# Shadowfear36/SegHiero

Measured on AMD Instinct MI355X. Metric: images/sec at 512x512 (ResNet-50 2-level), full train step, higher is better.
Workload: dtype f32 (convolutions: exact 3-way bf16 split of every fp32 operand, 6 bf16 MFMA products, f32 accumulate; rest plain f32)

## Files before the change

seghiero_amd/csrc/conv_bf16x6.hip:

```cpp
#include "conv_x6.h"

template <int MODE, int TM, int TN, int WGM, int WGN, int OCC = 0, int SK = 0, int PROF = 0, int ACT = 0>
__global__ __launch_bounds__(64 * WGM * WGN, OCC ? OCC : ((WGM * WGN) / 4 < 2 ? 2 : (WGM * WGN) / 4)) void conv_x6_kernel(const ConvQ p) {
    constexpr int NT = 64 * WGM * WGN;
    constexpr int BM = 32 * TM * WGM, BN = 32 * TN * WGN, BK = 32;
    constexpr int A_PLANE = BM * ROWB, B_PLANE = BN * ROWB;
    constexpr int RPP = NT / 8;
    constexpr int NA = (BM + RPP - 1) / RPP, NB = (BN + RPP - 1) / RPP;
    static_assert(BM >= RPP && BN >= RPP, "tile too small for the thread count");
    extern __shared__ __attribute__((aligned(16))) unsigned char smem[];

    const int t = threadIdx.x, lane = t & 63, wave = t >> 6;
    const int wm = wave / WGN, wn = wave % WGN, l31 = lane & 31, h = lane >> 5;
    unsigned long long tk0 = 0;
    if constexpr (PROF) tk0 = __builtin_amdgcn_s_memtime();
    const unsigned nblk = (unsigned)p.tiles_m * (unsigned)p.tiles_n;
    const unsigned bid = xcd_remap(blockIdx.x, nblk);
    const int tile_n = bid % p.tiles_n, tile_m = bid / p.tiles_n;
    const int m0 = tile_m * BM, n0 = tile_n * BN;
    int cy = 0, cx = 0, Hc = p.H, Wc = p.W, oy0 = 0, ox0 = 0, nth = p.KH, ntw = p.KW, Mc = p.M, Kt = p.K;
    if constexpr (MODE == DGRAD) {
        if (p.parity) {
            cy = blockIdx.y >> 1; cx = blockIdx.y & 1;
            oy0 = (cy + p.pad) & 1; ox0 = (cx + p.pad) & 1;
// ... 685 lines not shown
    const int tx = threadIdx.x & 31, ty = threadIdx.x >> 5;
    const float* w = T.w[lo];
    float* wt = T.wt[lo];
#pragma unroll
    for (int r = ty; r < 32; r += 8) {
        const int co = co0 + r, ci = ci0 + tx;
        tile[r][tx] = (co < Cout && ci < Cin) ? w[((long long)co * taps + tap) * Cin + ci] : 0.f;
    }
    __syncthreads();
#pragma unroll
    for (int r = ty; r < 32; r += 8) {
        const int ci = ci0 + r, co = co0 + tx;
        if (ci < Cin && co < CoutP) wt[((long long)tap * Cin + ci) * CoutP + co] = tile[tx][r];
    }
}
extern "C" int sh_weight_transpose_multi(int n, const float* const* w, float* const* wt, const int* cout, const int* taps, const int* cin,
                                         void* stream) {
    if (n <= 0 || n > SH_WT_MAX || !w || !wt || !cout || !taps || !cin) return SH_EINVAL;
    WtTab T;
    T.n = n;
    long long acc = 0;
    for (int i = 0; i < n; ++i) {
        if (!w[i] || !wt[i] || cout[i] <= 0 || taps[i] <= 0 || cin[i] <= 0) return SH_EINVAL;
        T.w[i] = w[i]; T.wt[i] = wt[i]; T.cout[i] = cout[i]; T.taps[i] = taps[i]; T.cin[i] = cin[i];
        T.start[i] = acc;
        acc += (long long)taps[i] * sh_cdiv((cout[i] + 3) & ~3, 32) * sh_cdiv(cin[i], 32);
    }
    T.start[n] = acc;
    if (acc >= (1ll << 31)) return SH_EINVAL;
    weight_transpose_multi_kernel<<<(unsigned)acc, 256, 0, (hipStream_t)stream>>>(T);
    return sh_launch_status();
}

struct BnbQ { const float* y; long long ldy; const float* mean; const float* invstd; const float* scale; const float* shift; int relu; const float* out; long long ldo;
              int act; int out_bf, add_bf; };
__global__ __launch_bounds__(256) void splitk_reduce_kernel(const float* __restrict__ slab, long long ldslab, int S, long long M, int Nn,
                                                            const float* __restrict__ bias, const float* __restrict__ addend, long long ldadd,
                                                            float* __restrict__ out, long long ldc, float* __restrict__ partials, const BnbQ bnb) {
    __shared__ float red[16][64];
    __shared__ float colmean[64];
    const int t = threadIdx.x, cq = t & 15, rl = t >> 4;
    const int n = blockIdx.y * 64 + cq * 4;
    const long long row0 = (long long)blockIdx.x * 64;
    const int npr = (int)(M - row0 < 64 ? M - row0 : 64);
    f32x4 v[4];
    const bool nok = n < Nn;
    f32x4 gq = {0.f, 0.f, 0.f, 0.f};
    f32x4 b_mu = gq, b_is = gq, b_sc = gq, b_sh = gq;
    if (bnb.y != nullptr && nok) { b_mu = ld4(bnb.mean + n); b_is = ld4(bnb.invstd + n); b_sc = ld4(bnb.scale + n); b_sh = ld4(bnb.shift + n); }
#pragma unroll
    for (int k = 0; k < 4; ++k) {
        const long long m = row0 + rl + 16 * k;
        v[k] = f32x4{0.f, 0.f, 0.f, 0.f};
        if (nok && m < M) {
            for (int s2 = 0; s2 < S; ++s2) v[k] += ld4(slab + ((long long)s2 * M + m) * ldslab + n);
            f32x4 o = v[k];
            if (bias) o += ld4(bias + n);
            if (addend) o += lda4(addend, m * ldadd + n, bnb.add_bf);
            if (bnb.y != nullptr) {
                const f32x4 yv = lda4(bnb.y, m * bnb.ldy + n, bnb.act & 4);
                if (bnb.relu) {
                    const f32x4 a = bnb.out == nullptr ? yv * b_sc + b_sh
                                    : ((bnb.act & 64) ? quad_mask_load(bnb.out, m * bnb.ldo + (n >> 2)) : lda4(bnb.out, m * bnb.ldo + n, bnb.act & 8));
#pragma unroll
                    for (int j = 0; j < 4; ++j) if (!(a[j] > 0.f)) o[j] = 0.f;
                }
                v[k] = o;
                gq += o * ((yv - b_mu) * b_is);
            }
            sta4(out, m * ldc + n, o, bnb.out_bf);
        }
    }
    if (partials == nullptr) return;
    f32x4 ssum = (v[0] + v[1]) + (v[2] + v[3]);
#pragma unroll
    for (int j = 0; j < 4; ++j) red[rl][cq * 4 + j] = ssum[j];
    __syncthreads();
    if (t < 64) {
        float a = 0.f;
#pragma unroll
        for (int k = 0; k < 16; ++k) a += red[k][t];
        colmean[t] = a / (float)npr;
        if (blockIdx.y * 64 + t < Nn) partials[((long long)blockIdx.x * 2 + 0) * Nn + blockIdx.y * 64 + t] = a;
    }
    __syncthreads();
    f32x4 q = {0.f, 0.f, 0.f, 0.f};
    if (bnb.y != nullptr) q = gq;
    else {
#pragma unroll
        for (int k = 0; k < 4; ++k)
            if (row0 + rl + 16 * k < M) {
#pragma unroll
                for (int j = 0; j < 4; ++j) { const float d = v[k][j] - colmean[cq * 4 + j]; q[j] += d * d; }
            }
    }
    __syncthreads();
#pragma unroll
    for (int j = 0; j < 4; ++j) red[rl][cq * 4 + j] = q[j];
    __syncthreads();
    if (t < 64 && blockIdx.y * 64 + t < Nn) {
        float a = 0.f;
#pragma unroll
        for (int k = 0; k < 16; ++k) a += red[k][t];
        partials[((long long)blockIdx.x * 2 + 1) * Nn + blockIdx.y * 64 + t] = a;
    }
}
int sh_x6_splitk_reduce(const ConvQ& p, int mode, hipStream_t st) {
    dim3 rg((unsigned)sh_cdiv(p.M, 64), (unsigned)sh_cdiv(p.Nn, 64));
    BnbQ bnb{p.bnb_y, p.bnb_ldy, p.bnb_mean, p.bnb_invstd, p.bnb_scale, p.bnb_shift, p.bnb_relu, p.bnb_out, p.bnb_ldo, mode == FPROP ? p.act : (p.act & ~2),
             mode == FPROP ? (p.act & 2) : (p.act & 128), mode == DGRAD ? (p.act & 256) : 0};
    splitk_reduce_kernel<<<rg, 256, 0, st>>>(p.slab, p.ldslab, p.ksplit, p.M, p.Nn, mode == FPROP ? p.extra : nullptr,
                                             mode == DGRAD ? p.extra : nullptr, p.ldadd, p.c, p.ldc,
                                             (mode == FPROP || p.bnb_y != nullptr) ? p.partials : nullptr, bnb);
    return sh_launch_status();
}
static int splitk_plan(long long M, long long N, long long K, int parity, int scatter, int b16 = 0) {
    if (parity || scatter || (N & 3)) return 1;
    const long long tiles = sh_cdiv(M, 128) * sh_cdiv(N, 128), nkt = sh_cdiv(K, 32);
    static int target6 = 0, minkt6 = 0, target1 = 0, minkt1 = 0;
    if (!target6) {
        const char* e = getenv("SEGHIERO_SK_TARGET"); target6 = e ? atoi(e) : 512; e = getenv("SEGHIERO_SK_MINKT"); minkt6 = e ? atoi(e) : 16;
        e = getenv("SEGHIERO_B16_SK_TARGET"); target1 = e ? atoi(e) : 1; e = getenv("SEGHIERO_B16_SK_MINKT"); minkt1 = e ? atoi(e) : 16;
    }
    const int target = b16 ? target1 : target6, minkt = b16 ? minkt1 : minkt6;
    if (tiles >= (target * 3) / 4 || nkt < 2 * minkt) return 1;
    long long S = sh_cdiv(target, tiles);
    if (S > nkt / minkt) S = nkt / minkt;
    if (S > 8) S = 8;
    return S < 2 ? 1 : (int)S;
}
template <int MODE, int TM, int TN, int WGM, int WGN, int OCC = 0, int SK = 0, int PROF = 0, int ACT = 0>
static int launch_x6(ConvQ& p, hipStream_t st) {
    constexpr int BM = 32 * TM * WGM, BN = 32 * TN * WGN;
    constexpr size_t lds = 3 * (size_t)(BM + BN) * ROWB;
    static bool attr_done = false;
    if (!attr_done) {
        (void)hipFuncSetAttribute(reinterpret_cast<const void*>(&conv_x6_kernel<MODE, TM, TN, WGM, WGN, OCC, SK, PROF, ACT>), hipFuncAttributeMaxDynamicSharedMemorySize, (int)lds);
        attr_done = true;
    }
    p.tiles_m = (int)sh_cdiv(p.M, BM);
    p.tiles_n = (int)sh_cdiv(p.Nn, BN);
    dim3 grid((unsigned)(p.tiles_m * p.tiles_n), p.parity ? 4u : (SK ? (unsigned)p.ksplit : 1u));
    conv_x6_kernel<MODE, TM, TN, WGM, WGN, OCC, SK, PROF, ACT><<<grid, 64 * WGM * WGN, lds, st>>>(p);
    if (SK) return sh_x6_splitk_reduce(p, MODE, st);
    return sh_launch_status();
}
static int x6_variant() { static int v = -1; if (v < 0) { const char* e = getenv("SEGHIERO_X6_VARIANT"); v = e ? atoi(e) : 0; } return v; }
template <int MODE>
static int launch_gemm_x6(ConvQ& p, hipStream_t st) {
    constexpr size_t lds = 2 * 3 * (size_t)(128 + 128) * ROWB_G;
    static bool attr_done = false;
    if (!attr_done) {
        (void)hipFuncSetAttribute(reinterpret_cast<const void*>(&gemm_x6_kernel<MODE>), hipFuncAttributeMaxDynamicSharedMemorySize, (int)lds);
        attr_done = true;
    }
    p.tiles_m = (int)sh_cdiv(p.M, 128);
    p.tiles_n = (int)sh_cdiv(p.Nn, 128);
    gemm_x6_kernel<MODE><<<(unsigned)(p.tiles_m * p.tiles_n), 256, lds, st>>>(p);
    return sh_launch_status();
}
template <int MODE>
static int launch_conv_x6(ConvQ& p, hipStream_t st) {
    const long long M = p.M, N = p.Nn;
    if (p.ksplit > 1) return launch_x6<MODE, 2, 2, 2, 2, 0, 1>(p, st);
    if (x6_variant() != 3 && p.KH * p.KW == 1 && p.stride == 1 && p.pad == 0 && !p.scatter && N >= 96 && p.K >= 1024 &&
        sh_cdiv(M, 128) * sh_cdiv(N, 128) >= 192) {
        p.ldb = (MODE == FPROP) ? p.K : p.Kc;
        return launch_gemm_x6<MODE>(p, st);
    }
    if (N > 128 && sh_cdiv(M, 256) * sh_cdiv(N, 256) >= 512) {
        if (sh_cdiv(N, 192) * 192 * 10 < sh_cdiv(N, 256) * 256 * 9) return launch_x6<MODE, 2, 2, 4, 3>(p, st);
        if (MODE == FPROP && x6_variant() == 7 && p.slab) return launch_x6<FPROP, 2, 2, 4, 4, 0, 0, 1>(p, st);
        return launch_x6<MODE, 2, 2, 4, 4>(p, st);
    }
    if (N > 64 && sh_cdiv(M, 256) * sh_cdiv(N, 128) >= 512) return launch_x6<MODE, 2, 2, 4, 2>(p, st);
    int TN = N <= 64 ? 1 : 2, TM = 2;
    if (sh_cdiv(M, 128) * sh_cdiv(N, 64 * TN) < 512) {
        TM = 1;
        if (TN == 2 && sh_cdiv(M, 64) * sh_cdiv(N, 128) < 512) TN = 1;
    }
    if (M <= 64) TM = 1;
    if (MODE == FPROP && TM == 2 && TN == 2 && x6_variant() == 7 && p.slab) return launch_x6<FPROP, 2, 2, 2, 2, 0, 0, 1>(p, st);
    if (TM == 2 && TN == 2) return launch_x6<MODE, 2, 2, 2, 2>(p, st);
    if (TM == 2 && TN == 1) return launch_x6<MODE, 2, 1, 2, 2>(p, st);
    if (TM == 1 && TN == 2) return launch_x6<MODE, 1, 2, 2, 2>(p, st);
    return launch_x6<MODE, 1, 1, 2, 2>(p, st);
}
static int launch_conv_x6_act(ConvQ& p, hipStream_t st) {
    const long long M = p.M, N = p.Nn;
    if (N > 128 && sh_cdiv(M, 256) * sh_cdiv(N, 256) >= 512) return launch_x6<FPROP, 2, 2, 4, 4, 0, 0, 0, 1>(p, st);
    int TN = N <= 64 ? 1 : 2, TM = 2;
    if (sh_cdiv(M, 128) * sh_cdiv(N, 64 * TN) < 512) {
        TM = 1;
        if (TN == 2 && sh_cdiv(M, 64) * sh_cdiv(N, 128) < 512) TN = 1;
    }
    if (M <= 64) TM = 1;
// ... 2 lines not shown
    if (TM == 1 && TN == 2) return launch_x6<FPROP, 1, 2, 2, 2, 0, 0, 0, 1>(p, st);
    return launch_x6<FPROP, 1, 1, 2, 2, 0, 0, 0, 1>(p, st);
}
static bool geom(ConvQ& p, int N, int H, int W, int Cin, int Cout, int KH, int KW, int stride, int pad, int dil) {
    if (N <= 0 || H <= 0 || W <= 0 || Cin <= 0 || Cout <= 0 || KH <= 0 || KW <= 0 || stride <= 0 || dil <= 0 || pad < 0) return false;
    if (Cin % 4 != 0) return false;
    p.N = N; p.H = H; p.W = W; p.Cin = Cin; p.Cout = Cout; p.KH = KH; p.KW = KW; p.stride = stride; p.pad = pad; p.dil = dil;
    p.Ho = (H + 2 * pad - dil * (KH - 1) - 1) / stride + 1;
    p.Wo = (W + 2 * pad - dil * (KW - 1) - 1) / stride + 1;
    if (p.Ho <= 0 || p.Wo <= 0) return false;
    if ((long long)N * H * W >= (1ll << 31) || (long long)N * p.Ho * p.Wo >= (1ll << 31)) return false;
    if ((long long)KH * KW * (long long)(Cin > Cout ? Cin : Cout + 3) >= (1ll << 30)) return false;
    return true;
}

extern "C" int64_t sh_conv_x6_workspace(int which, int N, int H, int W, int Cin, int Cout, int KH, int KW, int stride, int pad, int dil, int mode) {
    ConvQ p{};
    if (!geom(p, N, H, W, Cin, Cout, KH, KW, stride, pad, dil)) return -1;
    long long M, Nn, K;
    int parity = 0;
    if (which == 0) { M = (long long)N * p.Ho * p.Wo; Nn = Cout; K = (long long)KH * KW * Cin; }
    else {
        if (mode != 0) return 0;
        M = (long long)N * H * W; Nn = Cin; K = (long long)KH * KW * ((Cout + 3) & ~3);
        parity = stride == 2 && dil == 1 && KH * KW > 1;
    }
    const int S = splitk_plan(M, Nn, K, parity, 0);
    return S > 1 ? (int64_t)S * M * Nn * 4 : 0;
}
static void use_splitk(ConvQ& p, float* workspace, int64_t workspace_bytes, int b16 = 0) {
    if (x6_variant() == 7 && workspace && workspace_bytes >= (1 << 20)) { p.slab = workspace; return; }
    const int S = splitk_plan(p.M, p.Nn, p.K, p.parity, p.scatter, b16);
    if (S > 1 && workspace && workspace_bytes >= (int64_t)S * p.M * p.Nn * 4) { p.ksplit = S; p.slab = workspace; p.ldslab = p.Nn; }
}
static bool operand_extents(ConvQ& p, int mode) {
    long long a, b;
    if (mode == FPROP) { a = ((long long)p.N * p.H * p.W - 1) * p.lda + p.Cin; b = (long long)p.Cout * p.K; }
    else { a = ((long long)p.N * p.Ho * p.Wo - 1) * p.lda + p.Kc; b = (long long)p.KH * p.KW * p.Cin * p.Kc; }
    if (a * 4 >= (1ll << 31) || b * 4 >= (1ll << 31)) return false;
    p.a_bytes = (unsigned)(a * ((mode == FPROP && (p.act & 1)) ? 2 : 4)); p.b_bytes = (unsigned)(b * 4);
    return true;
}
static int launch_fprop_any(ConvQ& p, hipStream_t st) {
    if (operand_extents(p, FPROP)) { const int rc = sh_x6p_launch(FPROP, p, st); if (rc != SH_X6P_NO) return rc; }
    if (p.act) return SH_EUNSUPPORTED;
    return launch_conv_x6<FPROP>(p, st);
}
static int launch_dgrad_any(ConvQ& p, hipStream_t st) {
    if (operand_extents(p, DGRAD)) { const int rc = sh_x6p_launch(DGRAD, p, st); if (rc != SH_X6P_NO) return rc; }
    return launch_conv_x6<DGRAD>(p, st);
}
extern "C" int sh_conv_fprop_x6(const float* x, int ldx, const float* w, const float* bias, float* y, int ldy, float* stat_partials,
                                int N, int H, int W, int Cin, int Cout, int KH, int KW, int stride, int pad, int dil,
                                float* workspace, int64_t workspace_bytes, int act_flags, void* stream) {
    ConvQ p{};
    if (!x || !w || !y || !geom(p, N, H, W, Cin, Cout, KH, KW, stride, pad, dil)) return SH_EINVAL;
    if (ldx < Cin || ldy < Cout || (ldx & 3) || (act_flags & ~3)) return SH_EINVAL;
    p.act = act_flags;
    p.a = x; p.b = w; p.c = y; p.extra = bias; p.partials = stat_partials; p.lda = ldx; p.ldc = ldy;
    p.M = N * p.Ho * p.Wo; p.Nn = Cout; p.K = KH * KW * Cin; p.Kc = Cin;
    p.n_partials = (int)sh_cdiv(p.M, 64);
    if ((ldy & 3) == 0 && ((uintptr_t)y & 15) == 0 && (!bias || ((uintptr_t)bias & 15) == 0)) use_splitk(p, workspace, workspace_bytes);
    return launch_fprop_any(p, (hipStream_t)stream);
}
extern "C" int sh_conv_fprop_x6_aff(const float* x, int ldx, const float* in_scale, const float* in_shift, const float* w, const float* bias,
                                    float* y, int ldy, float* stat_partials, int N, int H, int W, int Cin, int Cout, int KH, int KW,
// ... 441 lines not shown
```

seghiero_amd/csrc/conv_x6.h:

```cpp
#pragma once
#include "common.h"
#include <stdlib.h>

enum { FPROP = 0, DGRAD = 1 };

struct ConvQ {
    const float* a;
    const float* b;
    float* c;
    const float* extra;
    float* partials;
    long long lda, ldb, ldc, ldadd;
    int N, H, W, Cin, Ho, Wo, Cout, KH, KW, stride, pad, dil;
    int M, Nn, K, Kc;
    int Kp;
    int Kreal;
    long long bplane;
    int scatter, sH, sW, sstride;
    int parity;
    int kchunk;
    int tiles_m, tiles_n, n_partials;
    const float* act_scale;
    const float* act_shift;
    const float* act_res;
// ... 46 lines not shown
    p1[0] = __builtin_amdgcn_perm(h1[1], h1[0], 0x07060302u); p1[1] = __builtin_amdgcn_perm(h1[3], h1[2], 0x07060302u);
    p2[0] = __builtin_amdgcn_perm(h2[1], h2[0], 0x07060302u); p2[1] = __builtin_amdgcn_perm(h2[3], h2[2], 0x07060302u);
    p3[0] = __builtin_amdgcn_perm(h3[1], h3[0], 0x07060302u); p3[1] = __builtin_amdgcn_perm(h3[3], h3[2], 0x07060302u);
}

#define ROWB 64
#define ROWB_G 80

__device__ __forceinline__ f32x16 mma6(const bf16x8 (&a)[3], const bf16x8 (&b)[3], f32x16 c) {
    c = mfma_bf16(a[2], b[0], c);
    c = mfma_bf16(a[0], b[2], c);
    c = mfma_bf16(a[1], b[1], c);
    c = mfma_bf16(a[1], b[0], c);
    c = mfma_bf16(a[0], b[1], c);
    c = mfma_bf16(a[0], b[0], c);
    return c;
}


__device__ __forceinline__ f32x16 mma3(const bf16x8 a0, const bf16x8 (&b)[3], f32x16 c) {
    c = mfma_bf16(a0, b[2], c);
    c = mfma_bf16(a0, b[1], c);
    c = mfma_bf16(a0, b[0], c);
    return c;
}

__device__ __forceinline__ f32x16 mma3b(const bf16x8 (&a)[3], const bf16x8 b0, f32x16 c) {
    c = mfma_bf16(a[2], b0, c);
    c = mfma_bf16(a[1], b0, c);
    c = mfma_bf16(a[0], b0, c);
    return c;
}

#define SH_X6P_NO (-100)
int sh_x6p_launch(int mode, ConvQ& p, hipStream_t st);
int sh_x6p_grouped_launch(ConvQ& p, hipStream_t st);
int sh_x6p_wgrad_launch(ConvQ& p, int wgm, int wgn, int splits, hipStream_t st);
int sh_b16_launch(int mode, ConvQ& p, int a32, hipStream_t st);
int sh_b16_grouped_launch(ConvQ& p, hipStream_t st);
int sh_b16_wgrad_launch(ConvQ& p, int dy32, int wgm, int wgn, int splits, hipStream_t st);
int sh_x6_splitk_reduce(const ConvQ& p, int mode, hipStream_t st);
```

seghiero_amd/csrc/conv_x6p.hip:

```cpp
#include "conv_x6.h"

__device__ __forceinline__ int swz_row(int row) { return ((row >> 2) & 3) ^ (row & 2); }

#ifndef SH_W1
#define SH_W1(AFF, EPI) ((AFF) == 2 ? 2 : 3)
#define SH_W2(AFF, EPI) (((AFF) == 2 || (EPI) == 2) ? 3 : 4)
#endif
#ifndef SH_X6P_PART
#define SH_X6P_PART 0
#endif
#define SH_PART(n) (SH_X6P_PART == 0 || SH_X6P_PART == (n))
int sh_x6p_launch_dgrad(ConvQ& p, hipStream_t st, int force);
int sh_x6p_wgrad_l0b0(ConvQ& p, bool aff, int wgm, int wgn, int splits, hipStream_t st);
int sh_x6p_wgrad_l1b0(ConvQ& p, bool aff, int wgm, int wgn, int splits, hipStream_t st);
int sh_x6p_wgrad_l0b1(ConvQ& p, bool aff, int wgm, int wgn, int splits, hipStream_t st);
int sh_x6p_wgrad_l1b1(ConvQ& p, bool aff, int wgm, int wgn, int splits, hipStream_t st);
static int x6p_mode() { static int v = -2; if (v == -2) { const char* e = getenv("SEGHIERO_X6P"); v = e ? atoi(e) : 1; } return v; }
[[maybe_unused]] static int x6p_ws() { static int v = -2; if (v == -2) { const char* e = getenv("SEGHIERO_X6P_WS"); v = e ? atoi(e) : 0; } return v; }
static int x6p_tile() { static int v = -2; if (v == -2) { const char* e = getenv("SEGHIERO_X6P_TILE"); v = e ? atoi(e) : 0; } return v; }
#if SH_PART(1) || SH_PART(2) || defined(SH_X6P_EXP)
template <int MODE, int TM, int TN, int WGM, int WGN, int WPS, int AFF, int EPI, int SK, int TAP, int GRP = 0, int ABF = 0, int WS = 0>
__global__ __launch_bounds__(64 * WGM * WGN * (WS ? 2 : 1), WPS) void conv_x6p_kernel(const ConvQ p) {
    constexpr int NT = 64 * WGM * WGN;
    constexpr int BM = 32 * TM * WGM, BN = 32 * TN * WGN;
    constexpr int A_PLANE = BM * ROWB, B_PLANE = BN * ROWB;
    constexpr int RPP = NT / 4;
    constexpr int NA = BM / RPP, NB = BN / RPP;
    static_assert(BM % RPP == 0 && BN % RPP == 0 && RPP % 64 == 0, "tile / thread-count mismatch");
    extern __shared__ __attribute__((aligned(16))) unsigned char smem[];
    unsigned char* const As = smem;
    unsigned char* const Bs = smem + 3 * A_PLANE;
    float* const coef = reinterpret_cast<float*>(smem + 3 * (A_PLANE + B_PLANE));
    static_assert(AFF != 2 || (MODE == DGRAD && TAP == 0 && !GRP), "the deferred BatchNorm-backward loader exists for 1x1 dgrads");
    static_assert(!ABF || (MODE == FPROP && !GRP) || AFF == 2, "bf16 loader streams: the fprop input, or the y stream of the lin loader");
    constexpr bool A_BF = ABF && MODE == FPROP, A2_BF = ABF && AFF == 2;
    constexpr bool A3 = A_BF && AFF == 0;
    auto load_a4 = [&](const __amdgpu_buffer_rsrc_t& rs, unsigned elem_off, unsigned ok, bool bf) -> f32x4 {
        if (bf) {
            const unsigned voff = ((elem_off * 2u) & ok) | (0x80000000u & ~ok);
            const u32x2 r = __builtin_bit_cast(u32x2, __builtin_amdgcn_raw_buffer_load_b64(rs, voff, 0, 0));
            return f32x4{__uint_as_float(r[0]), __uint_as_float(r[1]), 0.f, 0.f};
        }
        const unsigned voff = ((elem_off * 4u) & ok) | (0x80000000u & ~ok);
        return __builtin_bit_cast(f32x4, __builtin_amdgcn_raw_buffer_load_b128(rs, voff, 0, 0));
    };
    auto widen_a4 = [&](f32x4 v, bool bf) -> f32x4 {
        return bf ? bf16x4_to_f32(sh_u32x2{__float_as_uint(v[0]), __float_as_uint(v[1])}) : v;
    };

    const int t_all = threadIdx.x, t = WS ? (t_all & (NT - 1)) : t_all, lane = t & 63, wave = t >> 6;
    [[maybe_unused]] const bool producer = WS && t_all >= NT;
    static_assert(!WS || (NT & (NT - 1)) == 0, "wave-specialised form: power-of-two wave count");
    const int wm = wave / WGN, wn = wave % WGN, l31 = lane & 31, h = lane >> 5;
    const unsigned nblk = (unsigned)p.tiles_m * (unsigned)p.tiles_n;
    const unsigned bid = xcd_remap(blockIdx.x, nblk);
    const int tile_n = bid % p.tiles_n, tile_m = bid / p.tiles_n;
    const int m0 = tile_m * BM, n0 = tile_n * BN;
    const int grp = GRP ? n0 / p.group_n : 0;
    const float* const a_ptr = GRP ? p.ga[grp] : p.a;
    const float* const b_ptr = GRP ? p.gb[grp] : p.b;
    const unsigned a_bytes = GRP ? p.ga_bytes[grp] : p.a_bytes;
    const int lda = (int)(GRP ? p.glda[grp] : p.lda);
    const float* const sc_ptr = GRP ? p.gsc[grp] : p.aff_scale;
    const float* const sh_ptr = GRP ? p.gsh[grp] : p.aff_shift;
    const float aff_floor = (GRP && sc_ptr == nullptr) ? -INFINITY : 0.f;
    int cy = 0, cx = 0, Hc = p.H, Wc = p.W, oy0 = 0, ox0 = 0, ntw = p.KW, Mc = p.M, Kt = p.K;
    if constexpr (MODE == DGRAD) {
        if (p.parity) {
            cy = blockIdx.y >> 1; cx = blockIdx.y & 1;
            oy0 = (cy + p.pad) & 1; ox0 = (cx + p.pad) & 1;
            Hc = (p.H - oy0 + 1) >> 1; Wc = (p.W - ox0 + 1) >> 1;
            const int nth = (p.KH - cy + 1) >> 1;
            ntw = (p.KW - cx + 1) >> 1;
            Mc = p.N * Hc * Wc; Kt = nth * ntw * p.Kc;
            if (m0 >= Mc) return;
        }
    }
    int q_begin = 0, q_end = (Kt + 15) >> 4;
    if constexpr (SK) {
        const int per = ((q_end + p.ksplit - 1) / p.ksplit + 1) & ~1;
        q_begin = min(q_end, (int)blockIdx.y * per); q_end = min(q_end, q_begin + per);
    }
    const int klim = min(Kt, 16 * q_end);
    const int nq = (q_end - q_begin + 1) & ~1;
    constexpr bool single_tap = TAP == 0, tap_uniform = TAP <= 1;

    const __amdgpu_buffer_rsrc_t rsrc_a = __builtin_amdgcn_make_buffer_rsrc(const_cast<float*>(a_ptr), 0, a_bytes, 0x00020000);
    const __amdgpu_buffer_rsrc_t rsrc_b = __builtin_amdgcn_make_buffer_rsrc(const_cast<float*>(b_ptr), 0, p.b_bytes, 0x00020000);
    [[maybe_unused]] const __amdgpu_buffer_rsrc_t rsrc_a2 =
        __builtin_amdgcn_make_buffer_rsrc(const_cast<float*>(AFF == 2 ? p.a2 : a_ptr), 0, AFF == 2 ? p.a2_bytes : a_bytes, 0x00020000);
    constexpr unsigned OOB = 0x80000000u;
    const int kc = t & 3, r0 = t >> 2;
    int a_y[NA], a_x[NA], a_nb[NA];
    int b_row[NB];
    unsigned b_ok[NB];
    int cur_tap = -1;
    const bool direct = TAP == 0 && p.stride == 1 && p.pad == 0 && !(MODE == DGRAD && (p.parity || p.scatter));
#pragma unroll
    for (int i = 0; i < NA; ++i) {
        const int m = m0 + r0 + RPP * i;
        if (direct) { a_y[i] = m < Mc ? 0 : -(1 << 28); a_x[i] = 0; a_nb[i] = m < Mc ? m : 0; }
        else if (m < Mc) {
            if constexpr (MODE == FPROP) {
                const int ow = m % p.Wo, q = m / p.Wo, oh = q % p.Ho, n = q / p.Ho;
                a_y[i] = oh * p.stride - p.pad; a_x[i] = ow * p.stride - p.pad; a_nb[i] = n * p.H * p.W;
            } else {
                const int iwc = m % Wc, q = m / Wc, ihc = q % Hc, n = q / Hc;
                const int ih = p.parity ? 2 * ihc + oy0 : ihc, iw = p.parity ? 2 * iwc + ox0 : iwc;
                a_y[i] = ih + p.pad; a_x[i] = iw + p.pad; a_nb[i] = n * p.Ho * p.Wo;
            }
        } else { a_y[i] = -(1 << 28); a_x[i] = 0; a_nb[i] = 0; }
    }
#pragma unroll
    for (int i = 0; i < NB; ++i) {
        const int j = n0 + r0 + RPP * i;
        b_ok[i] = j < p.Nn ? ~0u : 0u;
        b_row[i] = (GRP ? j - grp * p.group_n : j) * (MODE == FPROP ? p.K : p.Kc);
// ... 137 lines not shown
#pragma unroll
        for (int i = 0; i < TM; ++i) {
            if constexpr (A3) {
                const bf16x8 a0 = __builtin_bit_cast(bf16x8, *reinterpret_cast<const u32x4*>(As + (arow + 32 * i) * ROWB + rd));
#pragma unroll
                for (int j = 0; j < TN; ++j) acc[i][j] = mma3(a0, bfr[j], acc[i][j]);
            } else {
            bf16x8 af[3];
#pragma unroll
            for (int pl = 0; pl < 3; ++pl)
                af[pl] = __builtin_bit_cast(bf16x8, *reinterpret_cast<const u32x4*>(As + pl * A_PLANE + (arow + 32 * i) * ROWB + rd));
#pragma unroll
            for (int j = 0; j < TN; ++j) acc[i][j] = mma6(af, bfr[j], acc[i][j]);
            }
        }
    };

    auto phase_schedule = [&]() {
        constexpr int PA = A3 ? 1 : 3, PP = A3 ? 3 : 6;
        constexpr int NMFMA = TM * TN * PP, NVALU = 30 * ((A3 ? 0 : NA) + NB) + (AFF == 2 ? 16 : 8 * AFF) * NA, NDSW = PA * NA + 3 * NB,
                      NVM = NA + NB + (AFF == 2 ? NA : 0);
        constexpr int VPM = (NVALU + NMFMA - 1) / NMFMA;
        __builtin_amdgcn_sched_group_barrier(0x100, 3 * TN + PA, 0);
#pragma unroll
        for (int g = 0; g < NMFMA; ++g) {
            __builtin_amdgcn_sched_group_barrier(0x008, 1, 0);
            __builtin_amdgcn_sched_group_barrier(0x002, VPM, 0);
            if (g * NDSW / NMFMA != (g + 1) * NDSW / NMFMA) __builtin_amdgcn_sched_group_barrier(0x200, 1, 0);
            if (g * NVM / NMFMA != (g + 1) * NVM / NMFMA) __builtin_amdgcn_sched_group_barrier(0x020, 1, 0);
            if (g % (PP * TN) == 2 && g / (PP * TN) + 1 < TM) __builtin_amdgcn_sched_group_barrier(0x100, PA, 0);
        }
    };
    if constexpr (AFF == 2) {
        for (int c = t_all; c < 4 * p.Kc; c += NT * (WS ? 2 : 1)) coef[c] = p.lin[c];
        __syncthreads();
    } else if constexpr (AFF) {
        for (int c = t_all; c < p.Kc; c += NT * (WS ? 2 : 1)) { coef[c] = sc_ptr ? sc_ptr[c] : 1.f; coef[p.Kc + c] = sh_ptr ? sh_ptr[c] : 0.f; }
        __syncthreads();
    }
    if constexpr (WS) {
        if (producer) {
            Regs R0, R1;
            prepare_tap(q_begin);     load_half(q_begin, R0);
            prepare_tap(q_begin + 1); load_half(q_begin + 1, R1);
            store_half(R0, 0);
            prepare_tap(q_begin + 2); load_half(q_begin + 2, R0);
            __syncthreads();
            for (int j = 0; j < nq; j += 2) {
                prepare_tap(q_begin + j + 3);
                store_half(R1, 1);
                load_half(q_begin + j + 3, R1);
                __syncthreads();
                prepare_tap(q_begin + j + 4);
                store_half(R0, 0);
                load_half(q_begin + j + 4, R0);
                __syncthreads();
            }
            return;
        }
        __syncthreads();
        for (int j = 0; j < nq; j += 2) {
            compute_half(0);
            __syncthreads();
            compute_half(1);
            __syncthreads();
        }
    } else {
    Regs R0, R1;
    prepare_tap(q_begin);     load_half(q_begin, R0);
    prepare_tap(q_begin + 1); load_half(q_begin + 1, R1);
// ... 2 lines not shown
    __syncthreads();
    for (int j = 0; j < nq; j += 2) {
        prepare_tap(q_begin + j + 3);
        store_half(R1, 1);
        load_half(q_begin + j + 3, R1);
        compute_half(0);
        phase_schedule();
        __syncthreads();
        prepare_tap(q_begin + j + 4);
        store_half(R0, 0);
        load_half(q_begin + j + 4, R0);
        compute_half(1);
        phase_schedule();
        __syncthreads();
    }
    }

    if constexpr (SK) {
        float* slab = p.slab + (long long)blockIdx.y * p.M * p.ldslab;
#pragma unroll
        for (int j = 0; j < TN; ++j) {
            const int n = n0 + wn * 32 * TN + 32 * j + l31;
#pragma unroll
            for (int i = 0; i < TM; ++i)
#pragma unroll
                for (int r = 0; r < 16; ++r) {
                    const int m = m0 + wm * 32 * TM + 32 * i + (r & 3) + 8 * (r >> 2) + 4 * h;
                    if (m < p.M && n < p.Nn) slab[(long long)m * p.ldslab + n] = acc[i][j][r];
                }
        }
        return;
    }

    static_assert(EPI == 0 || TM % 2 == 0, "statistics epilogues need whole 64-row groups per wave");
    int ncol[TN];
    bool nok[TN];
    float bias[TN];
    [[maybe_unused]] float b_mu[TN], b_is[TN], b_sc[TN], b_sh[TN];
#pragma unroll
    for (int j = 0; j < TN; ++j) {
        ncol[j] = n0 + wn * 32 * TN + 32 * j + l31;
        nok[j] = ncol[j] < p.Nn;
        bias[j] = (MODE == FPROP && p.extra != nullptr && nok[j]) ? p.extra[ncol[j]] : 0.f;
        if constexpr (EPI == 2) {
            b_mu[j] = b_is[j] = b_sc[j] = b_sh[j] = 0.f;
            if (nok[j]) { b_mu[j] = p.bnb_mean[ncol[j]]; b_is[j] = p.bnb_invstd[ncol[j]]; b_sc[j] = p.bnb_scale[ncol[j]]; b_sh[j] = p.bnb_shift[ncol[j]]; }
        }
    }
    if (EPI == 2 || p.vec_epi) {
        constexpr int WC = 32 * TN, RS = WC + 4, LPR = WC / 4, RPI = 64 / LPR, NRD = 32 / RPI;
        float* const stage = reinterpret_cast<float*>(smem) + wave * (32 * RS);
        const int rr = lane / LPR, c4 = (lane % LPR) * 4;
        const int ncv = n0 + wn * WC + c4;
        const bool nokv = ncv < p.Nn;
        f32x4 vb = zero4, v_mu = zero4, v_is = zero4, v_sc = zero4, v_sh = zero4;
        if (MODE == FPROP && p.extra != nullptr && nokv) vb = ld4(p.extra + ncv);
        if constexpr (EPI == 2) { if (nokv) { v_mu = ld4(p.bnb_mean + ncv); v_is = ld4(p.bnb_invstd + ncv); v_sc = ld4(p.bnb_scale + ncv); v_sh = ld4(p.bnb_shift + ncv); } }
        [[maybe_unused]] f32x4 pend_gs = zero4, pend_gq = zero4;
#pragma unroll
        for (int i = 0; i < TM; ++i) {
#pragma unroll
            for (int j = 0; j < TN; ++j)
#pragma unroll
                for (int r = 0; r < 16; ++r) stage[((r & 3) + 8 * (r >> 2) + 4 * h) * RS + 32 * j + l31] = acc[i][j][r];
            constexpr int CH = (EPI == 2 && NRD > 4) ? 4 : NRD;
            [[maybe_unused]] f32x4 gs = zero4, gq = zero4;
// ... 133 lines not shown
                const int prow0 = wrow0 + 64 * pr;
                const int npr = max(0, min(64, p.M - prow0));
                const int pidx = tile_m * (BM / 64) + wm * (TM / 2) + pr;
#pragma unroll
                for (int j = 0; j < TN; ++j) {
                    float ss = 0.f;
#pragma unroll
                    for (int i = 2 * pr; i < 2 * pr + 2; ++i)
#pragma unroll
                        for (int r = 0; r < 16; ++r) ss += acc[i][j][r];
                    ss += __shfl_xor(ss, 32, 64);
                    const float mean = npr > 0 ? ss / (float)npr : 0.f;
                    float qq = 0.f;
#pragma unroll
                    for (int i = 2 * pr; i < 2 * pr + 2; ++i)
#pragma unroll
                        for (int r = 0; r < 16; ++r) {
                            const int row = wrow0 + 32 * i + (r & 3) + 8 * (r >> 2) + 4 * h;
                            const float dv = acc[i][j][r] - mean;
                            qq += (npr == 64 || row < p.M) ? dv * dv : 0.f;
                        }
                    qq += __shfl_xor(qq, 32, 64);
                    const int n = n0 + wn * 32 * TN + 32 * j + l31;
                    if (h == 0 && pidx < p.n_partials && n < p.Nn) {
                        p.partials[((long long)pidx * 2 + 0) * p.Nn + n] = ss;
                        p.partials[((long long)pidx * 2 + 1) * p.Nn + n] = qq;
                    }
                }
            }
        }
    }
}

template <int MODE, int TM, int TN, int WGM, int WGN, int WPS, int AFF, int EPI, int SK, int TAP, int GRP = 0, int ABF = 0, int WS = 0>
static int launch_x6p(ConvQ& p, hipStream_t st) {
    constexpr int BM = 32 * TM * WGM, BN = 32 * TN * WGN;
    const size_t lds = 3 * (size_t)(BM + BN) * ROWB + (AFF == 2 ? 16 : AFF ? 8 : 0) * (size_t)p.Kc;
    if (lds > 160 * 1024) return SH_X6P_NO;
    static size_t attr_lds = 0;
    if (lds > attr_lds) {
        (void)hipFuncSetAttribute(reinterpret_cast<const void*>(&conv_x6p_kernel<MODE, TM, TN, WGM, WGN, WPS, AFF, EPI, SK, TAP, GRP, ABF, WS>),
                                  hipFuncAttributeMaxDynamicSharedMemorySize, (int)(160 * 1024));
        attr_lds = 160 * 1024;
    }
    p.tiles_m = (int)sh_cdiv(p.M, BM);
    p.tiles_n = (int)sh_cdiv(p.Nn, BN);
    dim3 grid((unsigned)(p.tiles_m * p.tiles_n), p.parity ? 4u : (SK ? (unsigned)p.ksplit : 1u));
    conv_x6p_kernel<MODE, TM, TN, WGM, WGN, WPS, AFF, EPI, SK, TAP, GRP, ABF, WS><<<grid, 64 * WGM * WGN * (WS ? 2 : 1), lds, st>>>(p);
    return sh_launch_status();
}

template <int MODE, int AFF, int EPI, int TAP, int ABF = 0>
static int pick_tile_x6p(ConvQ& p, hipStream_t st, int force) {
    (void)force;
    constexpr int W1 = SH_W1(AFF, EPI), W2 = SH_W2(AFF, EPI);
#ifdef SH_X6P_WS
    if (p.Nn > 64 && x6p_ws()) return launch_x6p<MODE, 2, 2, 2, 2, 2, AFF, EPI, 0, TAP, 0, ABF, 1>(p, st);
#endif
    if (p.Nn > 64) return launch_x6p<MODE, 2, 2, 2, 2, W1, AFF, EPI, 0, TAP, 0, ABF>(p, st);
    return launch_x6p<MODE, 2, 1, 2, 2, W2, AFF, EPI, 0, TAP, 0, ABF>(p, st);
}

template <int MODE, int AFF, int EPI, int ABF = 0>
static int pick_x6p(ConvQ& p, hipStream_t st, int force) {
    if constexpr (AFF == 2) {
        if (p.KH * p.KW != 1) return SH_X6P_NO;
        if (p.ksplit > 1) {
            const int rc = launch_x6p<MODE, 2, 2, 2, 2, 2, 2, 0, 1, 0, 0, ABF>(p, st);
            return rc == SH_OK ? sh_x6_splitk_reduce(p, MODE, st) : rc;
        }
        return pick_tile_x6p<MODE, 2, EPI, 0, ABF>(p, st, force);
    } else {
    if (p.ksplit > 1) {
        int rc;
        if (p.KH * p.KW == 1) rc = launch_x6p<MODE, 2, 2, 2, 2, 3, AFF, 0, 1, 0, 0, ABF>(p, st);
        else if ((p.Kc & 15) == 0) rc = launch_x6p<MODE, 2, 2, 2, 2, 3, AFF, 0, 1, 1, 0, ABF>(p, st);
        else return SH_X6P_NO;
        return rc == SH_OK ? sh_x6_splitk_reduce(p, MODE, st) : rc;
    }
    if (p.KH * p.KW == 1) return pick_tile_x6p<MODE, AFF, EPI, 0, ABF>(p, st, force);
    if ((p.Kc & 15) == 0) return pick_tile_x6p<MODE, AFF, EPI, 1, ABF>(p, st, force);
    if (AFF || EPI == 2 || ABF) return SH_X6P_NO;
    return pick_tile_x6p<MODE, 0, EPI, 2>(p, st, force);
    }
}

#endif
#if SH_PART(1)

int sh_x6p_grouped_launch(ConvQ& p, hipStream_t st) {
    if (p.ngroups < 1 || p.ngroups > 6 || (p.group_n & 127) || p.KH * p.KW != 1) return SH_X6P_NO;
    auto al16 = [](const void* q) { return ((uintptr_t)q & 15) == 0; };
    p.vec_epi = (p.ldc & 3) == 0 && al16(p.c);
    return launch_x6p<FPROP, 2, 2, 2, 2, 3, 1, 1, 0, 0, 1>(p, st);
}

int sh_x6p_launch(int mode, ConvQ& p, hipStream_t st) {
    const bool aff = p.aff_scale != nullptr, bnb = p.bnb_y != nullptr;
    if (!x6p_mode() && !aff && !bnb && !p.lin) return SH_X6P_NO;
    const int force = x6p_tile();
    auto al16 = [](const void* q) { return ((uintptr_t)q & 15) == 0; };
    p.vec_epi = !p.parity && !p.scatter && (p.Nn & 3) == 0 && (p.ldc & 3) == 0 && al16(p.c) &&
                (p.extra == nullptr || (al16(p.extra) && (mode == FPROP || (p.ldadd & 3) == 0))) &&
                (!bnb || ((p.bnb_ldy & 3) == 0 && al16(p.bnb_y) && (p.bnb_out == nullptr || (p.act & 64) || ((p.bnb_ldo & 3) == 0 && al16(p.bnb_out))) && al16(p.bnb_mean) && al16(p.bnb_invstd) && al16(p.bnb_scale) &&
                          al16(p.bnb_shift) && al16(p.partials)));
// ... 287 lines not shown
```

Before: 502.3.

## Split K across two wave groups inside one block, combine partials in LDS

Adds a K-group variant of the x6p conv kernel in which two four-wave groups in one 512-thread block each process half of the K range for the same 128x128 tile. The two partial accumulators are written to LDS and combined there by a shared split-K reduce body that also runs the BN/statistics epilogue. This replaces the global slab round-trip and the separate reduce kernel whenever the split-K plan picks two slices. Planning now also picks two slices when the workspace is too small for a slab. In exchange the block doubles its LDS use and runs at one block per SIMD group (WPS=1), and the epilogue goes through LDS serially.

```diff
diff --git a/seghiero_amd/csrc/conv_bf16x6.hip b/seghiero_amd/csrc/conv_bf16x6.hip
--- a/seghiero_amd/csrc/conv_bf16x6.hip
+++ b/seghiero_amd/csrc/conv_bf16x6.hip
@@ -741,83 +741,21 @@
     return sh_launch_status();
 }
 
-struct BnbQ { const float* y; long long ldy; const float* mean; const float* invstd; const float* scale; const float* shift; int relu; const float* out; long long ldo;
-              int act; int out_bf, add_bf; };
+struct GlobalSlab {
+    const float* slab; long long ldslab, M;
+    __device__ __forceinline__ f32x4 operator()(int s, long long m, int n) const { return ld4(slab + ((long long)s * M + m) * ldslab + n); }
+};
 __global__ __launch_bounds__(256) void splitk_reduce_kernel(const float* __restrict__ slab, long long ldslab, int S, long long M, int Nn,
                                                             const float* __restrict__ bias, const float* __restrict__ addend, long long ldadd,
                                                             float* __restrict__ out, long long ldc, float* __restrict__ partials, const BnbQ bnb) {
     __shared__ float red[16][64];
     __shared__ float colmean[64];
-    const int t = threadIdx.x, cq = t & 15, rl = t >> 4;
-    const int n = blockIdx.y * 64 + cq * 4;
-    const long long row0 = (long long)blockIdx.x * 64;
-    const int npr = (int)(M - row0 < 64 ? M - row0 : 64);
-    f32x4 v[4];
-    const bool nok = n < Nn;
-    f32x4 gq = {0.f, 0.f, 0.f, 0.f};
-    f32x4 b_mu = gq, b_is = gq, b_sc = gq, b_sh = gq;
-    if (bnb.y != nullptr && nok) { b_mu = ld4(bnb.mean + n); b_is = ld4(bnb.invstd + n); b_sc = ld4(bnb.scale + n); b_sh = ld4(bnb.shift + n); }
-#pragma unroll
-    for (int k = 0; k < 4; ++k) {
-        const long long m = row0 + rl + 16 * k;
-        v[k] = f32x4{0.f, 0.f, 0.f, 0.f};
-        if (nok && m < M) {
-            for (int s2 = 0; s2 < S; ++s2) v[k] += ld4(slab + ((long long)s2 * M + m) * ldslab + n);
-            f32x4 o = v[k];
-            if (bias) o += ld4(bias + n);
-            if (addend) o += lda4(addend, m * ldadd + n, bnb.add_bf);
-            if (bnb.y != nullptr) {
-                const f32x4 yv = lda4(bnb.y, m * bnb.ldy + n, bnb.act & 4);
-                if (bnb.relu) {
-                    const f32x4 a = bnb.out == nullptr ? yv * b_sc + b_sh
-                                    : ((bnb.act & 64) ? quad_mask_load(bnb.out, m * bnb.ldo + (n >> 2)) : lda4(bnb.out, m * bnb.ldo + n, bnb.act & 8));
-#pragma unroll
-                    for (int j = 0; j < 4; ++j) if (!(a[j] > 0.f)) o[j] = 0.f;
-                }
-                v[k] = o;
-                gq += o * ((yv - b_mu) * b_is);
-            }
-            sta4(out, m * ldc + n, o, bnb.out_bf);
-        }
-    }
-    if (partials == nullptr) return;
-    f32x4 ssum = (v[0] + v[1]) + (v[2] + v[3]);
-#pragma unroll
-    for (int j = 0; j < 4; ++j) red[rl][cq * 4 + j] = ssum[j];
-    __syncthreads();
-    if (t < 64) {
-        float a = 0.f;
-#pragma unroll
-        for (int k = 0; k < 16; ++k) a += red[k][t];
-        colmean[t] = a / (float)npr;
-        if (blockIdx.y * 64 + t < Nn) partials[((long long)blockIdx.x * 2 + 0) * Nn + blockIdx.y * 64 + t] = a;
-    }
-    __syncthreads();
-    f32x4 q = {0.f, 0.f, 0.f, 0.f};
-    if (bnb.y != nullptr) q = gq;
-    else {
-#pragma unroll
-        for (int k = 0; k < 4; ++k)
-            if (row0 + rl + 16 * k < M) {
-#pragma unroll
-                for (int j = 0; j < 4; ++j) { const float d = v[k][j] - colmean[cq * 4 + j]; q[j] += d * d; }
-            }
-    }
-    __syncthreads();
-#pragma unroll
-    for (int j = 0; j < 4; ++j) red[rl][cq * 4 + j] = q[j];
-    __syncthreads();
-    if (t < 64 && blockIdx.y * 64 + t < Nn) {
-        float a = 0.f;
-#pragma unroll
-        for (int k = 0; k < 16; ++k) a += red[k][t];
-        partials[((long long)blockIdx.x * 2 + 1) * Nn + blockIdx.y * 64 + t] = a;
-    }
+    splitk_reduce_body(GlobalSlab{slab, ldslab, M}, S, M, Nn, bias, addend, ldadd, out, ldc, partials, bnb, (int)threadIdx.x, (int)blockIdx.x,
+                       (int)blockIdx.y, red, colmean);
 }
 int sh_x6_splitk_reduce(const ConvQ& p, int mode, hipStream_t st) {
     dim3 rg((unsigned)sh_cdiv(p.M, 64), (unsigned)sh_cdiv(p.Nn, 64));
-    BnbQ bnb{p.bnb_y, p.bnb_ldy, p.bnb_mean, p.bnb_invstd, p.bnb_scale, p.bnb_shift, p.bnb_relu, p.bnb_out, p.bnb_ldo, mode == FPROP ? p.act : (p.act & ~2),
-             mode == FPROP ? (p.act & 2) : (p.act & 128), mode == DGRAD ? (p.act & 256) : 0};
+    const BnbQ bnb = bnbq_of(p, mode);
     splitk_reduce_kernel<<<rg, 256, 0, st>>>(p.slab, p.ldslab, p.ksplit, p.M, p.Nn, mode == FPROP ? p.extra : nullptr,
                                              mode == DGRAD ? p.extra : nullptr, p.ldadd, p.c, p.ldc,
                                              (mode == FPROP || p.bnb_y != nullptr) ? p.partials : nullptr, bnb);
@@ -871,6 +809,7 @@
 template <int MODE>
 static int launch_conv_x6(ConvQ& p, hipStream_t st) {
     const long long M = p.M, N = p.Nn;
+    if (p.ksplit > 1 && p.slab == nullptr) p.ksplit = 1;
     if (p.ksplit > 1) return launch_x6<MODE, 2, 2, 2, 2, 0, 1>(p, st);
     if (x6_variant() != 3 && p.KH * p.KW == 1 && p.stride == 1 && p.pad == 0 && !p.scatter && N >= 96 && p.K >= 1024 &&
         sh_cdiv(M, 128) * sh_cdiv(N, 128) >= 192) {
@@ -939,6 +878,7 @@
     if (x6_variant() == 7 && workspace && workspace_bytes >= (1 << 20)) { p.slab = workspace; return; }
     const int S = splitk_plan(p.M, p.Nn, p.K, p.parity, p.scatter, b16);
     if (S > 1 && workspace && workspace_bytes >= (int64_t)S * p.M * p.Nn * 4) { p.ksplit = S; p.slab = workspace; p.ldslab = p.Nn; }
+    else if (S == 2 && !b16 && workspace) p.ksplit = 2;
 }
 static bool operand_extents(ConvQ& p, int mode) {
     long long a, b;
diff --git a/seghiero_amd/csrc/conv_x6.h b/seghiero_amd/csrc/conv_x6.h
--- a/seghiero_amd/csrc/conv_x6.h
+++ b/seghiero_amd/csrc/conv_x6.h
@@ -102,6 +102,85 @@
     return c;
 }
 
+struct BnbQ { const float* y; long long ldy; const float* mean; const float* invstd; const float* scale; const float* shift; int relu; const float* out; long long ldo;
+              int act; int out_bf, add_bf; };
+__host__ __device__ __forceinline__ BnbQ bnbq_of(const ConvQ& p, int mode) {
+    return BnbQ{p.bnb_y, p.bnb_ldy, p.bnb_mean, p.bnb_invstd, p.bnb_scale, p.bnb_shift, p.bnb_relu, p.bnb_out, p.bnb_ldo, mode == FPROP ? p.act : (p.act & ~2),
+                mode == FPROP ? (p.act & 2) : (p.act & 128), mode == DGRAD ? (p.act & 256) : 0};
+}
+template <class Slab>
+__device__ __forceinline__ void splitk_reduce_body(const Slab& slab, int S, long long M, int Nn, const float* __restrict__ bias,
+                                                   const float* __restrict__ addend, long long ldadd, float* __restrict__ out, long long ldc,
+                                                   float* __restrict__ partials, const BnbQ& bnb, int t, int bx, int by,
+                                                   float (*red)[64], float* colmean) {
+    const int cq = t & 15, rl = t >> 4;
+    const int n = by * 64 + cq * 4;
+    const long long row0 = (long long)bx * 64;
+    const int npr = (int)(M - row0 < 64 ? M - row0 : 64);
+    const bool live = npr > 0;
+    f32x4 v[4];
+    const bool nok = n < Nn;
+    f32x4 gq = {0.f, 0.f, 0.f, 0.f};
+    f32x4 b_mu = gq, b_is = gq, b_sc = gq, b_sh = gq;
+    if (bnb.y != nullptr && nok) { b_mu = ld4(bnb.mean + n); b_is = ld4(bnb.invstd + n); b_sc = ld4(bnb.scale + n); b_sh = ld4(bnb.shift + n); }
+#pragma unroll
+    for (int k = 0; k < 4; ++k) {
+        const long long m = row0 + rl + 16 * k;
+        v[k] = f32x4{0.f, 0.f, 0.f, 0.f};
+        if (nok && m < M) {
+            for (int s2 = 0; s2 < S; ++s2) v[k] += slab(s2, m, n);
+            f32x4 o = v[k];
+            if (bias) o += ld4(bias + n);
+            if (addend) o += lda4(addend, m * ldadd + n, bnb.add_bf);
+            if (bnb.y != nullptr) {
+                const f32x4 yv = lda4(bnb.y, m * bnb.ldy + n, bnb.act & 4);
+                if (bnb.relu) {
+                    const f32x4 a = bnb.out == nullptr ? yv * b_sc + b_sh
+                                    : ((bnb.act & 64) ? quad_mask_load(bnb.out, m * bnb.ldo + (n >> 2)) : lda4(bnb.out, m * bnb.ldo + n, bnb.act & 8));
+#pragma unroll
+                    for (int j = 0; j < 4; ++j) if (!(a[j] > 0.f)) o[j] = 0.f;
+                }
+                v[k] = o;
+                gq += o * ((yv - b_mu) * b_is);
+            }
+            sta4(out, m * ldc + n, o, bnb.out_bf);
+        }
+    }
+    if (partials == nullptr) return;
+    f32x4 ssum = (v[0] + v[1]) + (v[2] + v[3]);
+#pragma unroll
+    for (int j = 0; j < 4; ++j) red[rl][cq * 4 + j] = ssum[j];
+    __syncthreads();
+    if (t < 64) {
+        float a = 0.f;
+#pragma unroll
+        for (int k = 0; k < 16; ++k) a += red[k][t];
+        colmean[t] = a / (float)npr;
+        if (live && by * 64 + t < Nn) partials[((long long)bx * 2 + 0) * Nn + by * 64 + t] = a;
+    }
+    __syncthreads();
+    f32x4 q = {0.f, 0.f, 0.f, 0.f};
+    if (bnb.y != nullptr) q = gq;
+    else {
+#pragma unroll
+        for (int k = 0; k < 4; ++k)
+            if (row0 + rl + 16 * k < M) {
+#pragma unroll
+                for (int j = 0; j < 4; ++j) { const float d = v[k][j] - colmean[cq * 4 + j]; q[j] += d * d; }
+            }
+    }
+    __syncthreads();
+#pragma unroll
+    for (int j = 0; j < 4; ++j) red[rl][cq * 4 + j] = q[j];
+    __syncthreads();
+    if (t < 64 && live && by * 64 + t < Nn) {
+        float a = 0.f;
+#pragma unroll
+        for (int k = 0; k < 16; ++k) a += red[k][t];
+        partials[((long long)bx * 2 + 1) * Nn + by * 64 + t] = a;
+    }
+}
+
 #define SH_X6P_NO (-100)
 int sh_x6p_launch(int mode, ConvQ& p, hipStream_t st);
 int sh_x6p_grouped_launch(ConvQ& p, hipStream_t st);
diff --git a/seghiero_amd/csrc/conv_x6p.hip b/seghiero_amd/csrc/conv_x6p.hip
--- a/seghiero_amd/csrc/conv_x6p.hip
+++ b/seghiero_amd/csrc/conv_x6p.hip
@@ -19,18 +19,22 @@
 [[maybe_unused]] static int x6p_ws() { static int v = -2; if (v == -2) { const char* e = getenv("SEGHIERO_X6P_WS"); v = e ? atoi(e) : 0; } return v; }
 static int x6p_tile() { static int v = -2; if (v == -2) { const char* e = getenv("SEGHIERO_X6P_TILE"); v = e ? atoi(e) : 0; } return v; }
 #if SH_PART(1) || SH_PART(2) || defined(SH_X6P_EXP)
-template <int MODE, int TM, int TN, int WGM, int WGN, int WPS, int AFF, int EPI, int SK, int TAP, int GRP = 0, int ABF = 0, int WS = 0>
-__global__ __launch_bounds__(64 * WGM * WGN * (WS ? 2 : 1), WPS) void conv_x6p_kernel(const ConvQ p) {
+template <int MODE, int TM, int TN, int WGM, int WGN, int WPS, int AFF, int EPI, int SK, int TAP, int GRP = 0, int ABF = 0, int WS = 0, int KG = 1>
+__global__ __launch_bounds__(64 * WGM * WGN * (WS ? 2 : 1) * KG, WPS) void conv_x6p_kernel(const ConvQ p) {
     constexpr int NT = 64 * WGM * WGN;
+    constexpr int NTB = NT * (WS ? 2 : 1) * KG;
+    static_assert(KG == 1 || (KG == 2 && !SK && !WS && !GRP && EPI == 0 && TM == 2 && TN == 2 && WGM == 2 && WGN == 2),
+                  "K groups: two four-wave groups on one 128 x 128 tile, epilogue by splitk_reduce_body");
     constexpr int BM = 32 * TM * WGM, BN = 32 * TN * WGN;
     constexpr int A_PLANE = BM * ROWB, B_PLANE = BN * ROWB;
     constexpr int RPP = NT / 4;
     constexpr int NA = BM / RPP, NB = BN / RPP;
     static_assert(BM % RPP == 0 && BN % RPP == 0 && RPP % 64 == 0, "tile / thread-count mismatch");
     extern __shared__ __attribute__((aligned(16))) unsigned char smem[];
-    unsigned char* const As = smem;
-    unsigned char* const Bs = smem + 3 * A_PLANE;
-    float* const coef = reinterpret_cast<float*>(smem + 3 * (A_PLANE + B_PLANE));
+    const int kgrp = KG == 2 ? __builtin_amdgcn_readfirstlane((int)(threadIdx.x / NT)) : 0;
+    unsigned char* const As = smem + kgrp * (3 * (A_PLANE + B_PLANE));
+    unsigned char* const Bs = As + 3 * A_PLANE;
+    float* const coef = reinterpret_cast<float*>(smem + KG * 3 * (A_PLANE + B_PLANE));
     static_assert(AFF != 2 || (MODE == DGRAD && TAP == 0 && !GRP), "the deferred BatchNorm-backward loader exists for 1x1 dgrads");
     static_assert(!ABF || (MODE == FPROP && !GRP) || AFF == 2, "bf16 loader streams: the fprop input, or the y stream of the lin loader");
     constexpr bool A_BF = ABF && MODE == FPROP, A2_BF = ABF && AFF == 2;
@@ -48,9 +52,9 @@
         return bf ? bf16x4_to_f32(sh_u32x2{__float_as_uint(v[0]), __float_as_uint(v[1])}) : v;
     };
 
-    const int t_all = threadIdx.x, t = WS ? (t_all & (NT - 1)) : t_all, lane = t & 63, wave = t >> 6;
+    const int t_all = threadIdx.x, t = (WS || KG == 2) ? (t_all & (NT - 1)) : t_all, lane = t & 63, wave = t >> 6;
     [[maybe_unused]] const bool producer = WS && t_all >= NT;
-    static_assert(!WS || (NT & (NT - 1)) == 0, "wave-specialised form: power-of-two wave count");
+    static_assert((!WS && KG == 1) || (NT & (NT - 1)) == 0, "wave-specialised form / K groups: power-of-two wave count");
     const int wm = wave / WGN, wn = wave % WGN, l31 = lane & 31, h = lane >> 5;
     const unsigned nblk = (unsigned)p.tiles_m * (unsigned)p.tiles_n;
     const unsigned bid = xcd_remap(blockIdx.x, nblk);
@@ -77,12 +81,15 @@
         }
     }
     int q_begin = 0, q_end = (Kt + 15) >> 4;
-    if constexpr (SK) {
-        const int per = ((q_end + p.ksplit - 1) / p.ksplit + 1) & ~1;
-        q_begin = min(q_end, (int)blockIdx.y * per); q_end = min(q_end, q_begin + per);
+    int nq_long = 0;
+    if constexpr (SK || KG == 2) {
+        const int nsl = KG == 2 ? 2 : p.ksplit, sl = KG == 2 ? kgrp : (int)blockIdx.y;
+        const int per = ((q_end + nsl - 1) / nsl + 1) & ~1;
+        nq_long = (min(q_end, per) + 1) & ~1;
+        q_begin = min(q_end, sl * per); q_end = min(q_end, q_begin + per);
     }
     const int klim = min(Kt, 16 * q_end);
-    const int nq = (q_end - q_begin + 1) & ~1;
+    const int nq = KG == 2 ? nq_long : ((q_end - q_begin + 1) & ~1);
     constexpr bool single_tap = TAP == 0, tap_uniform = TAP <= 1;
 
     const __amdgpu_buffer_rsrc_t rsrc_a = __builtin_amdgcn_make_buffer_rsrc(const_cast<float*>(a_ptr), 0, a_bytes, 0x00020000);
@@ -286,10 +293,10 @@
         }
     };
     if constexpr (AFF == 2) {
-        for (int c = t_all; c < 4 * p.Kc; c += NT * (WS ? 2 : 1)) coef[c] = p.lin[c];
+        for (int c = t_all; c < 4 * p.Kc; c += NTB) coef[c] = p.lin[c];
         __syncthreads();
     } else if constexpr (AFF) {
-        for (int c = t_all; c < p.Kc; c += NT * (WS ? 2 : 1)) { coef[c] = sc_ptr ? sc_ptr[c] : 1.f; coef[p.Kc + c] = sh_ptr ? sh_ptr[c] : 0.f; }
+        for (int c = t_all; c < p.Kc; c += NTB) { coef[c] = sc_ptr ? sc_ptr[c] : 1.f; coef[p.Kc + c] = sh_ptr ? sh_ptr[c] : 0.f; }
         __syncthreads();
     }
     if constexpr (WS) {
@@ -358,6 +365,43 @@
         return;
     }
 
+    if constexpr (KG == 2) {
+        static_assert(TM == 2, "a wave row owns one 64-row half of the tile");
+        constexpr int LDR = BN + 4;
+        float* const img = reinterpret_cast<float*>(smem);
+        float* const mine = img + kgrp * (64 * LDR);
+        struct LdsSlab {
+            const float* img; int m0, n0;
+            __device__ __forceinline__ f32x4 operator()(int s, long long m, int n) const {
+                return *reinterpret_cast<const f32x4*>(img + s * (64 * LDR) + ((int)m - m0) * LDR + (n - n0));
+            }
+        };
+        const int team = kgrp;
+        float* const scratch = img + KG * (64 * LDR) + team * (16 * 64 + 64);
+        float (*const red)[64] = reinterpret_cast<float (*)[64]>(scratch);
+        float* const colmean = scratch + 16 * 64;
+        const BnbQ bnb = bnbq_of(p, MODE);
+#pragma unroll
+        for (int s = 0; s < BM / 64; ++s) {
+            if (wm == s) {
+#pragma unroll
+                for (int i = 0; i < TM; ++i)
+#pragma unroll
+                    for (int j = 0; j < TN; ++j)
+#pragma unroll
+                        for (int r = 0; r < 16; ++r)
+                            mine[(32 * i + (r & 3) + 8 * (r >> 2) + 4 * h) * LDR + wn * 32 * TN + 32 * j + l31] = acc[i][j][r];
+            }
+            __syncthreads();
+            splitk_reduce_body(LdsSlab{img, m0 + 64 * s, n0}, 2, (long long)p.M, p.Nn, MODE == FPROP ? p.extra : nullptr,
+                               MODE == DGRAD ? p.extra : nullptr, p.ldadd, p.c, p.ldc,
+                               (MODE == FPROP || p.bnb_y != nullptr) ? p.partials : nullptr, bnb, t,
+                               tile_m * (BM / 64) + s, tile_n * (BN / 64) + team, red, colmean);
+            __syncthreads();
+        }
+        return;
+    }
+
     static_assert(EPI == 0 || TM % 2 == 0, "statistics epilogues need whole 64-row groups per wave");
     int ncol[TN];
     bool nok[TN];
@@ -557,21 +601,22 @@
     }
 }
 
-template <int MODE, int TM, int TN, int WGM, int WGN, int WPS, int AFF, int EPI, int SK, int TAP, int GRP = 0, int ABF = 0, int WS = 0>
+template <int MODE, int TM, int TN, int WGM, int WGN, int WPS, int AFF, int EPI, int SK, int TAP, int GRP = 0, int ABF = 0, int WS = 0, int KG = 1>
 static int launch_x6p(ConvQ& p, hipStream_t st) {
     constexpr int BM = 32 * TM * WGM, BN = 32 * TN * WGN;
-    const size_t lds = 3 * (size_t)(BM + BN) * ROWB + (AFF == 2 ? 16 : AFF ? 8 : 0) * (size_t)p.Kc;
+    const size_t lds = KG * 3 * (size_t)(BM + BN) * ROWB + (AFF == 2 ? 16 : AFF ? 8 : 0) * (size_t)p.Kc;
+    static_assert(KG == 1 || (size_t)(2 * 64 * (BN + 4) + 2 * (16 * 64 + 64)) * sizeof(float) <= KG * 3 * (size_t)(BM + BN) * ROWB, "combine images fit the planes");
     if (lds > 160 * 1024) return SH_X6P_NO;
     static size_t attr_lds = 0;
     if (lds > attr_lds) {
-        (void)hipFuncSetAttribute(reinterpret_cast<const void*>(&conv_x6p_kernel<MODE, TM, TN, WGM, WGN, WPS, AFF, EPI, SK, TAP, GRP, ABF, WS>),
+        (void)hipFuncSetAttribute(reinterpret_cast<const void*>(&conv_x6p_kernel<MODE, TM, TN, WGM, WGN, WPS, AFF, EPI, SK, TAP, GRP, ABF, WS, KG>),
                                   hipFuncAttributeMaxDynamicSharedMemorySize, (int)(160 * 1024));
         attr_lds = 160 * 1024;
     }
     p.tiles_m = (int)sh_cdiv(p.M, BM);
     p.tiles_n = (int)sh_cdiv(p.Nn, BN);
     dim3 grid((unsigned)(p.tiles_m * p.tiles_n), p.parity ? 4u : (SK ? (unsigned)p.ksplit : 1u));
-    conv_x6p_kernel<MODE, TM, TN, WGM, WGN, WPS, AFF, EPI, SK, TAP, GRP, ABF, WS><<<grid, 64 * WGM * WGN * (WS ? 2 : 1), lds, st>>>(p);
+    conv_x6p_kernel<MODE, TM, TN, WGM, WGN, WPS, AFF, EPI, SK, TAP, GRP, ABF, WS, KG><<<grid, 64 * WGM * WGN * (WS ? 2 : 1) * KG, lds, st>>>(p);
     return sh_launch_status();
 }
 
@@ -590,12 +635,24 @@
 static int pick_x6p(ConvQ& p, hipStream_t st, int force) {
     if constexpr (AFF == 2) {
         if (p.KH * p.KW != 1) return SH_X6P_NO;
+        if (p.ksplit == 2) {
+            const int rc = launch_x6p<MODE, 2, 2, 2, 2, 1, 2, 0, 0, 0, 0, ABF, 0, 2>(p, st);
+            if (rc != SH_X6P_NO) return rc;
+            if (p.slab == nullptr) p.ksplit = 1;
+        }
         if (p.ksplit > 1) {
             const int rc = launch_x6p<MODE, 2, 2, 2, 2, 2, 2, 0, 1, 0, 0, ABF>(p, st);
             return rc == SH_OK ? sh_x6_splitk_reduce(p, MODE, st) : rc;
         }
         return pick_tile_x6p<MODE, 2, EPI, 0, ABF>(p, st, force);
     } else {
+    if (p.ksplit == 2) {
+        int rc = SH_X6P_NO;
+        if (p.KH * p.KW == 1) rc = launch_x6p<MODE, 2, 2, 2, 2, 1, AFF, 0, 0, 0, 0, ABF, 0, 2>(p, st);
+        else if ((p.Kc & 15) == 0) rc = launch_x6p<MODE, 2, 2, 2, 2, 1, AFF, 0, 0, 1, 0, ABF, 0, 2>(p, st);
+        if (rc != SH_X6P_NO) return rc;
+        if (p.slab == nullptr) p.ksplit = 1;
+    }
     if (p.ksplit > 1) {
         int rc;
         if (p.KH * p.KW == 1) rc = launch_x6p<MODE, 2, 2, 2, 2, 3, AFF, 0, 1, 0, 0, ABF>(p, st);
```

New measurement: 504.1, median of 6. About the same (+0.4%).
